# xarray-contrib/xeofs

Hardware: AMD Instinct MI355X
Metric: EOF randomized-SVD GB/s (algorithmic: 16 passes x n x p x 4 B per fit / fit time) (higher is better)
Workload: dtype f32 data, split-fp16 MFMA (f16x3+f16x3), f32 accumulate

## Files before the change

xeofs_amd/csrc/eofx_abi.hip:

```cpp
#include <chrono>
#include "eofx_hfft.hpp"
#include "eofx_kernels.hpp"
#include "eofx_fit.hpp"
#include "eofx_gram.hpp"
#include "eofx_axb_dma.hpp"
#include "eofx_hosteig.hpp"
#include "eofx_hostla.hpp"
#include "eofx_lag.hpp"
#include "eofx_gw.hpp"
#include "eofx_spca.hpp"
#include "eofx_lagcov.hpp"
#include "eofx_lowpass.hpp"
#include "eofx_orderpos.hpp"
#include "eofx_colquad.hpp"
#include "eofx_pairmin.hpp"
#include "eofx_simplex.hpp"
#include "eofx_spectral.hpp"
#include "eofx_pcmul.hpp"
#include "eofx_viewcov.hpp"
#include "eofx_lrfill.hpp"
#include "eofx_plans.hpp"
#include "eofx_sketch.hpp"
#include "eofx_hilbert_host.hpp"
#include "eofx_gwplan.hpp"
// ... 806 lines not shown
#undef EOFX_AXB_ARGS
    KCHK();
  }
  if (ctx->profile) {
    HIPCHK(hipEventRecord(ev1, ctx->stream));
    ctx->prof_events.emplace_back(ev0, ev1, 1);
    ctx->prof_flops += 2.0 * (double)K * (double)rows_pad * (double)L;
    ctx->prof_bytes += (double)K * (double)rows * 4.0 * tiles.columns();
  }
  if (plan.S > 1) {
    const int64_t count4 = rows_pad * L / 4;
    hipLaunchKernelGGL(splitk_reduce_kernel, dim3((int)std::min<int64_t>((count4 + 255) / 256, amax_out ? 2048 : 4096)), dim3(256), 0,
                       ctx->stream, out, W, count4, plan.S, amax_out);
    KCHK();
  }
  return EOFX_OK;
}

static int launch_gram(eofx_ctx* ctx, const float* P, int64_t rows, int L, double* G) {
  const int nb = (L + 63) / 64;
  const int nbx = gram_parts(rows, L);
  ArenaScope scope(ctx);
  ARENA(double, part, (size_t)nbx * L * L);
  hipLaunchKernelGGL(gram_mfma_kernel, dim3(nbx, nb * nb), dim3(256), 0, ctx->stream, P, rows, L, part);
  KCHK();
  const int64_t count = (int64_t)L * L;
  hipLaunchKernelGGL(f64_reduce_kernel, dim3((int)((count + 63) / 64)), dim3(256), 0, ctx->stream,
                     part, G, count, nbx);
  KCHK();
  return EOFX_OK;
}
static int launch_matmul(eofx_ctx* ctx, const float* P, int64_t rows, int L, const double* Mx, int Lo,
                         float* out, bool upper = false, int64_t planes_rows = 0, float planes_bound = 0.f) {
  int KW = (int)std::min<int64_t>(round_up(L, 64), 256);
  if (L > 256) {
    static const int kw_env = std::getenv("EOFX_PMM_KW") ? atoi(std::getenv("EOFX_PMM_KW")) : 0;
    if (kw_env == 128 || kw_env == 256) KW = kw_env;
  }
  const size_t smem = (size_t)KW * PMM_LD * sizeof(double);
  if (smem > 64 * 1024)
    HIPCHK(hipFuncSetAttribute(reinterpret_cast<const void*>(panel_matmul_kernel<false>), hipFuncAttributeMaxDynamicSharedMemorySize, (int)smem));
  const int64_t units = (rows + 127) / 128;
  const int64_t gx = L <= KW ? std::min<int64_t>(units, 1024) : units;
  dim3 grid((int)std::max<int64_t>(1, gx), (Lo + 63) / 64);
  unsigned* amax_out = amax_new(ctx, out);
  if (planes_rows > 0 && Lo == L && amax_out && planes_rows % AXB_KG == 0 && planes_rows <= rows && rows % 8 == 0 && planes_bound > 0.f &&
      std::isfinite(planes_bound) && axb_planes_reserve(ctx, axb_planes_bytes(planes_rows, Lo))) {
    if (smem > 64 * 1024)
      HIPCHK(hipFuncSetAttribute(reinterpret_cast<const void*>(panel_matmul_kernel<false, true>), hipFuncAttributeMaxDynamicSharedMemorySize,
                                 (int)smem));
    hipLaunchKernelGGL((panel_matmul_kernel<false, true>), grid, dim3(256), smem, ctx->stream, P, rows, L, Mx, Lo, out, KW, amax_out,
                       (int64_t)0, (int64_t)0, 1, (const float*)nullptr, upper ? 1 : 0, ctx->axb_planes, planes_rows, planes_bound);
    KCHK();
    ctx->planes_known.panel = out;
    ctx->planes_known.L = Lo;
    ctx->planes_known.K_all = planes_rows;
    ctx->planes_known.bound = planes_bound;
    ctx->planes_known.f32 = true;
    ++ctx->plane_produced[1];
    return EOFX_OK;
  }
  hipLaunchKernelGGL(panel_matmul_kernel<false>, grid, dim3(256), smem, ctx->stream, P, rows, L, Mx, Lo, out, KW, amax_out,
                     (int64_t)0, (int64_t)0, 1, (const float*)nullptr, upper ? 1 : 0);
  KCHK();
  return EOFX_OK;
}
static int launch_matmul_gen(eofx_ctx* ctx, const float* P, int64_t ldp, int64_t slab, int cpb, int64_t rows, int L, const double* Mx, int Lo,
                             const float* sub, float* out) {
  const int KW = (int)std::min<int64_t>(round_up(L, 64), 256);
  const size_t smem = (size_t)KW * PMM_LD * sizeof(double);
  if (smem > 64 * 1024)
    HIPCHK(hipFuncSetAttribute(reinterpret_cast<const void*>(panel_matmul_kernel<true>), hipFuncAttributeMaxDynamicSharedMemorySize, (int)smem));
  const int64_t units = (rows + 127) / 128;
  const int64_t gx = L <= KW ? std::min<int64_t>(units, 1024) : units;
  dim3 grid((int)std::max<int64_t>(1, gx), (Lo + 63) / 64);
  hipLaunchKernelGGL(panel_matmul_kernel<true>, grid, dim3(256), smem, ctx->stream, P, rows, L, Mx, Lo, out, KW, amax_new(ctx, out), ldp,
                     slab, cpb, sub);
  KCHK();
  return EOFX_OK;
}
static int launch_xgram(eofx_ctx* ctx, const float* Pa, int64_t lda, int La, const float* Pb, int64_t ldb, int Lb, int64_t rows, double* C) {
  const int nbx = (int)std::max<int64_t>(1, std::min<int64_t>((rows + 127) / 128, std::max<int64_t>(1, ((int64_t)32 << 20) / ((int64_t)La * Lb * 8))));
  ArenaScope scope(ctx);
  ARENA(double, part, (size_t)nbx * La * Lb);
  hipLaunchKernelGGL(xgram_mfma_kernel, dim3(nbx, (La / 64) * (Lb / 64)), dim3(256), 0, ctx->stream, Pa, lda, Pb, ldb, rows, La, Lb, part);
  KCHK();
// ... 981 lines not shown
    return set_err(ctx, EOFX_ERR_ARG, "import: L=%d must be a positive multiple of 4, l=%d and rows=%lld non-negative", L, l, (long long)rows);
  ENTER(ctx);
  CHK(arena_reserve(ctx, (size_t)rows * l * sizeof(float) + 8192));
  return import_panel(ctx, src, rows, l, P, rows_pad, L);
}

struct LinOp {
  int64_t tall, small, tall_pad, small_pad;
  std::function<int(const float*, float*, int, int)> fwd;
  std::function<int(const float*, float*, int, int)> bwd;
  std::function<int(const float*, float*, int, int, bool)> fwd_to_bwd;
  std::function<int64_t(int, int)> bwd_plane_rows;
  std::function<int(double*, int64_t)> reduce_tall_gram;
  std::function<int(double*, int64_t)> reduce_small_gram;
  int64_t rule_tall_pad = 0;
};

struct RsvdOut {
  float* Tvec;
  float* Svec;
  int Lo;
  std::vector<double> s;
  int64_t tall_pad = 0, small_pad = 0;
};

extern "C" int eofx_orth_tall_rule(int64_t tall_rows_pad, int L, int prec_power) {
  return orth_tall_rule(tall_rows_pad, L, prec_power) ? 1 : 0;
}
extern "C" int eofx_peaked_spectrum(const double* G, int ld, int l) {
  if (!G || l <= 0) return 0;
  std::vector<double> A((size_t)l * l), w(l), V((size_t)l * l);
  for (int i = 0; i < l; ++i)
    for (int j = 0; j < l; ++j) A[(size_t)i * l + j] = 0.5 * (G[(size_t)i * ld + j] + G[(size_t)j * ld + i]);
  for (double v : A)
    if (!std::isfinite(v)) return 0;
  if (eofx_host_eigh_f64(A.data(), l, w.data(), V.data()) != EOFX_OK) return 1;
  if (!(w[0] > 0.0)) return 0;
  return hostla::peaked_spectrum(w.data(), l) ? 1 : 0;
}

static int launch_rinv_blocked(eofx_ctx* ctx, const double* G, int L, int l, double* Rinv) {
  const int Lb = (int)round_up(l, 64), nb = Lb / 64;
  ArenaScope scope(ctx);
  ARENA(double, S, (size_t)Lb * Lb);
  ARENA(double, X, (size_t)Lb * Lb);
  ARENA(double, T, (size_t)Lb * Lb / 2 + 64 * 64);
// ... 74 lines not shown
  }
  return EOFX_OK;
}

constexpr int EOFX_FIT_FALLBACK = 1;
typedef std::function<int(const float*, float*, int)> FirstFwd;
typedef std::function<int(const float*, float*, int)> RangeFinder;
static int rsvd_core(eofx_ctx* ctx, const LinOp& op, int k, int l, int n_iter, const float* omega,
                     RsvdOut& out, const FirstFwd* first_fwd = nullptr, const RangeFinder* range = nullptr) {
  const int L = (int)round_up(l, 32);
  const int Lo = (int)round_up(k, 32);
  AmaxScope amax_scope(ctx);
  ARENA(float, Zs, (size_t)op.small_pad * L);
  ARENA(float, Ws, (size_t)op.small_pad * L);
  ARENA(float, Yt, (size_t)op.tall_pad * L);
  ARENA(float, Qt, (size_t)op.tall_pad * L);
  ARENA(float, Tv, (size_t)op.tall_pad * Lo);
  ARENA(float, Sv, (size_t)op.small_pad * Lo);
  ARENA(double, G, (size_t)L * L);
  ARENA(double, G0, (size_t)L * L);
  ARENA(double, R2, (size_t)L * L);
  ARENA(double, Md, (size_t)L * Lo);
  ARENA(double, Md2, (size_t)L * Lo);
  double* pin = nullptr;
  CHK(pinned_scratch(ctx, &pin));
  if ((size_t)2 * L * L > EOFX_PINNED_DOUBLES) return set_err(ctx, EOFX_ERR_ARG, "internal: sketch too wide for the host scratch");

  CHK(import_panel(ctx, omega, op.small, l, Zs, op.small_pad, L));
  bool first_done = false;
  auto fwd = [&](const float* z, float* y, int prec, int to_bwd = 0) -> int {
    if (first_fwd && !first_done) {
      first_done = true;
      return (*first_fwd)(z, y, L);
    }
    first_done = true;
    if (to_bwd && op.fwd_to_bwd) return op.fwd_to_bwd(z, y, L, prec, to_bwd == 1);
    return op.fwd(z, y, L, prec);
  };
  auto gram_tall = [&](const float* Pn, double* Gout) -> int {
    CHK(launch_gram(ctx, Pn, op.tall_pad, L, Gout));
    return op.reduce_tall_gram ? op.reduce_tall_gram(Gout, (int64_t)L * L) : EOFX_OK;
  };
  auto gram_small = [&](const float* Pn, double* Gout) -> int {
    CHK(launch_gram(ctx, Pn, op.small_pad, L, Gout));
    return op.reduce_small_gram ? op.reduce_small_gram(Gout, (int64_t)L * L) : EOFX_OK;
  };
// ... 61 lines not shown
                       "SVD failed. This may be due to isolated NaN values in the data.");
      Gl[(size_t)i * l + j] = v;
    }
  eofx_host_eigh_f64(Gl.data(), l, w.data(), Uh.data());
  out.s.assign(k, 0.0);
  std::vector<double> M1((size_t)L * Lo, 0.0), M2((size_t)L * Lo, 0.0);
  std::vector<double> invs(k);
  for (int j = 0; j < k; ++j) {
    const double sv = std::sqrt(std::max(w[j], 0.0));
    out.s[j] = sv;
    invs[j] = sv > 0.0 ? 1.0 / sv : 0.0;
  }
  for (int i = 0; i < l; ++i) {
    double* m1 = &M1[(size_t)i * Lo];
    for (int q = 0; q < l; ++q) {
      const double r = hR2[(size_t)i * L + q];
      const double* uq = &Uh[(size_t)q * l];
      for (int j = 0; j < k; ++j) m1[j] += r * uq[j];
    }
    for (int j = 0; j < k; ++j) M2[(size_t)i * Lo + j] = Uh[(size_t)i * l + j] * invs[j];
  }
  HIPCHK(hipMemcpyAsync(Md, M1.data(), sizeof(double) * L * Lo, hipMemcpyHostToDevice, ctx->stream));
  HIPCHK(hipMemcpyAsync(Md2, M2.data(), sizeof(double) * L * Lo, hipMemcpyHostToDevice, ctx->stream));
  CHK(launch_matmul(ctx, Qt, op.tall_pad, L, Md, Lo, Tv));
  CHK(launch_matmul(ctx, Ws, op.small_pad, L, Md2, Lo, Sv));
  HIPCHK(hipStreamSynchronize(ctx->stream));
  out.Tvec = Tv;
  out.Svec = Sv;
  out.Lo = Lo;
  out.tall_pad = op.tall_pad;
  out.small_pad = op.small_pad;
  return EOFX_OK;
}

static int comm_allreduce(eofx_ctx* ctx, void* buf, int64_t count, int dtype, int op);
static int sign_rule(eofx_ctx* ctx, const float* Vpanel, int64_t rows, int Lo, int k,
                     std::vector<double>& sign, bool over_ranks = false) {
  ArenaScope scope(ctx);
  ARENA(float, mx, 2 * (size_t)Lo);
  float* mn = mx + Lo;
  CHK(launch_colminmax(ctx, Vpanel, rows, Lo, mx, mn));
  if (over_ranks) {
    hipLaunchKernelGGL(negate_kernel, dim3(1), dim3(256), 0, ctx->stream, mn, Lo);
    KCHK();
    CHK(comm_allreduce(ctx, mx, 2 * (int64_t)Lo, 0, 1));
  }
  std::vector<float> hmx(Lo), hmn(Lo);
  HIPCHK(hipMemcpyAsync(hmx.data(), mx, sizeof(float) * Lo, hipMemcpyDeviceToHost, ctx->stream));
  HIPCHK(hipMemcpyAsync(hmn.data(), mn, sizeof(float) * Lo, hipMemcpyDeviceToHost, ctx->stream));
  HIPCHK(hipStreamSynchronize(ctx->stream));
  sign.assign(k, 1.0);
  for (int j = 0; j < k; ++j) sign[j] = (std::fabs(hmx[j]) >= std::fabs(hmn[j])) ? 1.0 : -1.0;
  return EOFX_OK;
}

typedef std::function<int(double*, int64_t)> GramReduce;
static int fix_null_columns(eofx_ctx* ctx, float* P, int64_t rows, int64_t rows_pad, int Lo, int k, int first,
                            const GramReduce* reduce = nullptr, int64_t rows_total = -1) {
  if (rows_total < 0) rows_total = rows;
  if (first >= k || rows_total <= first) return EOFX_OK;
  if (!reduce) {
    if (ctx->arena_size - ctx->arena_off < null_repair_bytes(rows_pad, Lo)) return EOFX_OK;
  }
  ArenaScope scope(ctx);
  ARENA(double, G, (size_t)Lo * Lo);
  ARENA(double, Mx, (size_t)Lo * Lo);
  ARENA(float, tmp, (size_t)rows_pad * Lo);
  ARENA(int, dflag, Lo);
  std::vector<double> hG((size_t)Lo * Lo), hM((size_t)Lo * Lo);
  std::vector<int> flag(Lo, 0);
  const int blocks = (int)std::max<int64_t>(1, std::min<int64_t>((rows + 255) / 256, 4096));
  auto gram = [&]() -> int {
    CHK(launch_gram(ctx, P, rows_pad, Lo, G));
// ... 10 lines not shown
    return EOFX_OK;
  };
  int rounds_done = 0;
  for (int attempt = 0; attempt < 8 && rounds_done < 2; ++attempt) {
    CHK(gram());
    const int verdict = hostla::null_column_transform(hG.data(), Lo, first, k, rounds_done == 0, hM.data(), flag.data());
    if (verdict != hostla::NULLCOL_OK) {
      if (rounds_done > 0) break;
      CHK(refill());
      continue;
    }
    HIPCHK(hipMemcpyAsync(Mx, hM.data(), sizeof(double) * Lo * Lo, hipMemcpyHostToDevice, ctx->stream));
    CHK(launch_matmul(ctx, P, rows_pad, Lo, Mx, Lo, tmp));
    HIPCHK(hipMemcpy2DAsync(P + first, sizeof(float) * Lo, tmp + first, sizeof(float) * Lo, sizeof(float) * (size_t)(k - first), (size_t)rows_pad,
                            hipMemcpyDeviceToDevice, ctx->stream));
    HIPCHK(hipStreamSynchronize(ctx->stream));
    ++rounds_done;
  }
  return EOFX_OK;
}

static int fix_null_modes(eofx_ctx* ctx, const RsvdOut& ro, int64_t tall, int64_t small, int k,
                          const GramReduce* reduce_tall = nullptr, int64_t tall_total = -1,
                          const GramReduce* reduce_small = nullptr, int64_t small_total = -1) {
  int first_null = k;
  const double s0 = ro.s.empty() ? 0.0 : ro.s[0];
  for (int j = k - 1; j >= 0 && !(ro.s[j] > 1e-5 * s0); --j) first_null = j;
  if (first_null < k && s0 >= 0.0 && std::isfinite(s0) && ro.tall_pad >= tall && ro.small_pad >= small) {
    CHK(fix_null_columns(ctx, ro.Tvec, tall, ro.tall_pad, ro.Lo, k, first_null, reduce_tall, tall_total));
    CHK(fix_null_columns(ctx, ro.Svec, small, ro.small_pad, ro.Lo, k, first_null, reduce_small, small_total));
  }
  return EOFX_OK;
}

struct FactorShards {
  const GramReduce* reduce_tall = nullptr;
  int64_t tall_total = -1;
  const GramReduce* reduce_small = nullptr;
  int64_t small_total = -1;
};
static int rsvd_finish(eofx_ctx* ctx, const RsvdOut& ro, bool right_is_tall, int64_t left_rows, int64_t right_rows, int k, int flip,
                       float* left, float* s, float* right, double s_divisor = 1.0, const FactorShards* shards = nullptr,
                       std::vector<double>* sign_out = nullptr) {
  const int64_t tall = right_is_tall ? right_rows : left_rows, small = right_is_tall ? left_rows : right_rows;
  const FactorShards local, &sh = shards ? *shards : local;
  CHK(fix_null_modes(ctx, ro, tall, small, k, sh.reduce_tall, sh.tall_total, sh.reduce_small, sh.small_total));
  const float* Rp = right_is_tall ? ro.Tvec : ro.Svec;
  const float* Lp = right_is_tall ? ro.Svec : ro.Tvec;
  std::vector<double> sign;
  if (flip) CHK(sign_rule(ctx, Rp, right_rows, ro.Lo, k, sign, shards != nullptr));
  CHK(export_panel(ctx, Lp, left_rows, ro.Lo, k, flip ? sign.data() : nullptr, left));
  CHK(export_panel(ctx, Rp, right_rows, ro.Lo, k, flip ? sign.data() : nullptr, right));
  if (s) {
    std::vector<float> hs(k);
    for (int j = 0; j < k; ++j) hs[j] = (float)(ro.s[j] / s_divisor);
    HIPCHK(hipMemcpy(s, hs.data(), sizeof(float) * k, hipMemcpyDefault));
  }
  HIPCHK(hipStreamSynchronize(ctx->stream));
  if (sign_out) sign_out->swap(sign);
  return EOFX_OK;
}

static const float* identity_sketch(int64_t small, int l, std::vector<float>& eye) {
  eye.assign((size_t)small * l, 0.f);
  for (int64_t i = 0; i < l; ++i) eye[(size_t)i * l + i] = 1.f;
  return eye.data();
}

extern "C" int eofx_rsvd_f32(eofx_ctx* ctx, const eofx_mat* m, int k, int n_oversamples, int n_iter,
                             const float* omega, int flip, float* U, float* s, float* V) {
  if (!ctx || !m || !omega || k <= 0 || n_oversamples < 0) return set_err(ctx, EOFX_ERR_ARG, "bad argument");
  ENTER(ctx);
  const int64_t n = m->n, p = m->p;
// ... 3523 lines not shown
```

xeofs_amd/csrc/eofx_kernels.hpp:

```cpp
#pragma once
#include <hip/hip_runtime.h>
#include <stdint.h>

#include "eofx_mfma64.hpp"
#include "eofx_plans.hpp"

namespace eofx {

typedef float f32x16 __attribute__((ext_vector_type(16)));
typedef float f32x4 __attribute__((ext_vector_type(4)));
typedef float f32x2 __attribute__((ext_vector_type(2)));

__device__ __forceinline__ void aff_split(double sh, float& hi, float& lo) {
  hi = (float)sh;
  lo = (float)(sh - (double)hi);
}
__device__ __forceinline__ float aff_map(float x, float sh_hi, float sh_lo, float scale) {
  return ((x - sh_hi) - sh_lo) * scale;
}
__device__ __forceinline__ float aff_fma(float x, float sh_hi, float s, float nls) {
  return __builtin_fmaf(x - sh_hi, s, nls);
}

__device__ __forceinline__ void amax_commit(float mx, unsigned* __restrict__ amax_out) {
// ... 968 lines not shown
    f32x4 o = {(float)s0, (float)s1, (float)s2, (float)s3};
    reinterpret_cast<f32x4*>(out)[i] = o;
    mx = fmaxf(mx, fmaxf(fmaxf(fabsf(o[0]), fabsf(o[1])), fmaxf(fabsf(o[2]), fabsf(o[3]))));
  }
  if (amax_out) amax_commit(mx, amax_out);
}

__global__ __launch_bounds__(256) void symmetrize_lower_kernel(float* __restrict__ C, int64_t n, int64_t ld) {
  __shared__ float T[64][65];
  const int bi = blockIdx.y, bj = blockIdx.x;
  if (bj > bi) return;
  const int tx = threadIdx.x & 63, ty = threadIdx.x >> 6;
  for (int r = ty; r < 64; r += 4) {
    const int64_t gr = (int64_t)bj * 64 + r, gc = (int64_t)bi * 64 + tx;
    T[r][tx] = (gr < n && gc < n) ? C[gr * ld + gc] : 0.f;
  }
  __syncthreads();
  for (int r = ty; r < 64; r += 4) {
    const int64_t gr = (int64_t)bi * 64 + r, gc = (int64_t)bj * 64 + tx;
    if (gr < n && gc < n && gc < gr) C[gr * ld + gc] = T[tx][r];
  }
}

__global__ __launch_bounds__(256) void gram_mfma_kernel(const float* __restrict__ P, int64_t rows, int L,
                                                         double* __restrict__ Gpart) {
  const int nb = (L + 63) / 64;
  const int bi = blockIdx.y / nb, bj = blockIdx.y % nb;
  if (bi > bj) return;
  const int wave = threadIdx.x >> 6;
  const Mfma64Lane ln = mfma64_lane();
  const int ca = 64 * bi + 4 * ln.c, cb = 64 * bj + 4 * ln.c;
  const bool same = (bi == bj);
  f64x4 acc[4][4];
  mfma64_zero(acc);
  const int64_t wstride = (int64_t)gridDim.x * 4 * 4;
  auto fetch = [&](int64_t r0, f32x4& va, f32x4& vb) {
    const int64_t r = r0 + ln.k;
    va = f32x4{0.f, 0.f, 0.f, 0.f};
    vb = va;
    if (r < rows) {
      if (ca < L) va = *reinterpret_cast<const f32x4*>(P + r * L + ca);
      if (!same && cb < L) vb = *reinterpret_cast<const f32x4*>(P + r * L + cb);
    }
    if (same) vb = va;
  };
  constexpr int GRAM_PF = 4;
  int64_t r0 = ((int64_t)blockIdx.x * 4 + wave) * 4;
  f32x4 pa[GRAM_PF], pb[GRAM_PF];
#pragma unroll
  for (int d = 0; d < GRAM_PF; ++d) fetch(r0 + d * wstride, pa[d], pb[d]);
  for (; r0 < rows; r0 += GRAM_PF * wstride) {
#pragma unroll
    for (int d = 0; d < GRAM_PF; ++d) {
      const f32x4 va = pa[d], vb = pb[d];
      fetch(r0 + (GRAM_PF + d) * wstride, pa[d], pb[d]);
      __builtin_amdgcn_sched_barrier(0);
      const double a[4] = {(double)va[0], (double)va[1], (double)va[2], (double)va[3]};
      const double b[4] = {(double)vb[0], (double)vb[1], (double)vb[2], (double)vb[3]};
      if (same)
        mfma64_step(acc, a, b, [](int x, int y) { return y >= x; });
      else
        mfma64_step(acc, a, b, Mfma64All{});
    }
  }
  __shared__ double Gs[64][65];
  for (int w = 0; w < 4; ++w) {
    if (wave == w)
      mfma64_each_interleaved(acc, [&](int x, int y) { return !(same && x > y); },
                              [&](int x, int y, int i, int j, double v) {
                                if (w == 0) {
                                  Gs[i][j] = v;
                                  if (same && x < y) Gs[j][i] = v;
                                } else {
                                  Gs[i][j] += v;
                                  if (same && x < y) Gs[j][i] += v;
                                }
                              });
    __syncthreads();
  }
  double* G = Gpart + (int64_t)blockIdx.x * (int64_t)L * L;
  for (int e = threadIdx.x; e < 64 * 64; e += 256) {
    const int i = e >> 6, j = e & 63;
    const int gi = 64 * bi + i, gj = 64 * bj + j;
    if (gi < L && gj < L) {
      G[(int64_t)gi * L + gj] = Gs[i][j];
// ... 281 lines not shown
}

__global__ void chol_blocked_init_kernel(const double* __restrict__ G, int L, int l, double* __restrict__ S, int Lb,
                                          double* __restrict__ d0) {
  const int64_t total = (int64_t)Lb * Lb;
  for (int64_t i = (int64_t)blockIdx.x * blockDim.x + threadIdx.x; i < total; i += (int64_t)gridDim.x * blockDim.x) {
    const int r = (int)(i / Lb), c = (int)(i % Lb);
    double v = (r == c) ? 1.0 : 0.0;
    if (r < l && c < l) v = G[(int64_t)r * L + c];
    S[i] = v;
    if (r == c) d0[r] = v;
  }
}
__global__ void chol_blocked_export_kernel(const double* __restrict__ X, int Lb, int l, double* __restrict__ Rinv, int L) {
  const int64_t total = (int64_t)L * L;
  for (int64_t i = (int64_t)blockIdx.x * blockDim.x + threadIdx.x; i < total; i += (int64_t)gridDim.x * blockDim.x) {
    const int r = (int)(i / L), c = (int)(i % L);
    Rinv[i] = (r <= c && c < l) ? X[(int64_t)r * Lb + c] : 0.0;
  }
}

constexpr int PMM_LD = 66;

template <bool GEN = false, bool PLANES = false>
__global__ __launch_bounds__(256) void panel_matmul_kernel(const float* __restrict__ P,
                                                           int64_t rows, int L,
                                                           const double* __restrict__ Mx, int Lo,
                                                           float* __restrict__ out, int KW,
                                                           unsigned* __restrict__ amax_out = nullptr,
                                                           int64_t ldp = 0, int64_t slab = 0, int cpb = 1,
                                                           const float* __restrict__ sub = nullptr, int upper = 0,
                                                           void* __restrict__ planes = nullptr, int64_t plane_rows = 0,
                                                           float plane_bound = 0.f) {
  static_assert(!(GEN && PLANES), "the plane epilogue belongs to the plain form");
  extern __shared__ __attribute__((aligned(16))) double Ms[];
  float amx = 0.f;
  const int tid = threadIdx.x;
  const int lane = tid & 63, wave = tid >> 6;
  const int li = lane & 15, lk = lane >> 4;
  const int by = upper ? (int)(gridDim.y - 1 - blockIdx.y) : (int)blockIdx.y;
  const int c0 = by * 64;
  const int Lc_all = (L + 63) / 64;
  const int Lc = upper ? (Lc_all < by + 1 ? Lc_all : by + 1) : Lc_all;
  const int Le = L < 64 * Lc ? L : 64 * Lc;
  const int64_t ngroups = (rows + 31) / 32;
  const int64_t g0 = (int64_t)blockIdx.x * 4 + wave;
  auto stage = [&](int k0) {
    for (int i = tid; i < KW * 64; i += 256) {
      const int r = i >> 6, c = i & 63;
      Ms[r * PMM_LD + c] = (k0 + r < L && c0 + c < Lo) ? Mx[(int64_t)(k0 + r) * Lo + c0 + c] : 0.0;
    }
  };
  auto fetch = [&](bool valid, int64_t g, int kc, f32x4 (&a)[2][4]) {
#pragma unroll
    for (int t = 0; t < 2; ++t) {
      const int64_t r = 32 * g + (PLANES ? 8 * (li & 3) + 4 * t + (li >> 2) : 16 * t + li);
#pragma unroll
      for (int tt = 0; tt < 4; ++tt) {
        const int k = kc + 16 * tt + 4 * lk;
        if constexpr (GEN)
          a[t][tt] = (valid && r < rows && k < L) ? *reinterpret_cast<const f32x4*>(P + (int64_t)((k >> 6) / cpb) * slab + ((k >> 6) % cpb) * 64 + r * ldp + (k & 63))
                                                 : f32x4{0.f, 0.f, 0.f, 0.f};
        else
          a[t][tt] = (valid && r < rows && k < L) ? *reinterpret_cast<const f32x4*>(P + r * L + k)
                                                 : f32x4{0.f, 0.f, 0.f, 0.f};
      }
    }
  };
  f64x4 acc[2][4];
  auto compute = [&](int64_t g, int kc, int ms0, const f32x4 (&a)[2][4]) {
    if (kc == 0) {
#pragma unroll
      for (int t = 0; t < 2; ++t)
#pragma unroll
        for (int q = 0; q < 4; ++q) acc[t][q] = f64x4{0.0, 0.0, 0.0, 0.0};
    }
#pragma unroll
    for (int tt = 0; tt < 4; ++tt)
#pragma unroll
      for (int c = 0; c < 4; ++c) {
        double b[4];
#pragma unroll
        for (int q = 0; q < 4; ++q) b[q] = Ms[(kc - ms0 + 16 * tt + 4 * lk + c) * PMM_LD + 16 * q + li];
#pragma unroll
        for (int t = 0; t < 2; ++t)
#pragma unroll
          for (int q = 0; q < 4; ++q)
            acc[t][q] = __builtin_amdgcn_mfma_f64_16x16x4f64((double)a[t][tt][c], b[q], acc[t][q], 0, 0, 0);
      }
    if (kc + 64 >= Le) {
#pragma unroll
      for (int t = 0; t < 2; ++t)
#pragma unroll
        for (int r = 0; r < 4; ++r) {
          const int64_t row = 32 * g + (PLANES ? 8 * lk + 4 * t + r : 16 * t + lk + 4 * r);
          if (row >= rows) continue;
#pragma unroll
          for (int q = 0; q < 4; ++q) {
            const int col = c0 + 16 * q + li;
            if (col < Lo) {
              float o_ = (float)acc[t][q][r];
              if constexpr (GEN) {
                if (sub) o_ = (float)((double)sub[row * Lo + col] - acc[t][q][r]);
              }
              out[row * Lo + col] = o_;
              amx = fmaxf(amx, fabsf(o_));
            }
          }
        }
      if constexpr (PLANES) {
        const int64_t k = 32 * g + 8 * lk;
        if (k < plane_rows) {
          const float p_scale = f16_scale_for(plane_bound);
          float m1 = -1.f;
          asm volatile("" : "+v"(m1));
#pragma unroll
          for (int q = 0; q < 4; ++q) {
            const int col = c0 + 16 * q + li;
            u32x4 hi, lo;
#pragma unroll
            for (int t = 0; t < 2; ++t)
#pragma unroll
              for (int r = 0; r < 4; r += 2) {
                const bool in_ = col < Lo && k + 4 * t + r < rows;
                const float v0 = (in_ ? (float)acc[t][q][r] : 0.f) * p_scale;
                const float v1 = (in_ ? (float)acc[t][q][r + 1] : 0.f) * p_scale;
                const fp16x2_t h = cvt_pk_rn(v0, v1);
                fp16x2_t l;
                l[0] = (__fp16)__builtin_fmaf((float)h[0], m1, v0);
// ... 23 lines not shown
      if (item + 1 < nitems) {
        fetch(item + 2 < nitems, g0 + ((item + 2) / Lc) * gstride, (int)((item + 2) % Lc) * 64, a0);
        __builtin_amdgcn_sched_barrier(0);
        compute(g0 + ((item + 1) / Lc) * gstride, (int)((item + 1) % Lc) * 64, 0, a1);
      }
    }
  } else {
    const bool active = g0 < ngroups;
    const int wc = KW / 64;
    fetch(active, g0, 0, a0);
    for (int w0 = 0; w0 < Lc; w0 += wc) {
      __syncthreads();
      stage(64 * w0);
      __syncthreads();
      const int we = w0 + wc < Lc ? w0 + wc : Lc;
      for (int ch = w0; ch < we; ch += 2) {
        fetch(active && ch + 1 < Lc, g0, 64 * (ch + 1), a1);
        __builtin_amdgcn_sched_barrier(0);
        if (active) compute(g0, 64 * ch, 64 * w0, a0);
        fetch(active && ch + 2 < Lc, g0, 64 * (ch + 2), a0);
        __builtin_amdgcn_sched_barrier(0);
        if (active && ch + 1 < we) compute(g0, 64 * (ch + 1), 64 * w0, a1);
      }
    }
  }
  if constexpr (PLANES) {
    if (amax_out && blockIdx.x == 0 && blockIdx.y == 0 && tid == 0) *amax_out = __float_as_uint(plane_bound);
  } else if (amax_out) {
    amax_commit(amx, amax_out);
  }
}

__global__ __launch_bounds__(256) void colminmax_part_kernel(const float* __restrict__ P,
                                                             int64_t rows, int L,
                                                             float* __restrict__ pmx,
                                                             float* __restrict__ pmn) {
  __shared__ float smx[16][64], smn[16][64];
  const int tid = threadIdx.x;
  const int cq = tid & 15, rl = tid >> 4;
  const int c = blockIdx.y * 64 + 4 * cq;
  f32x4 mx = {-INFINITY, -INFINITY, -INFINITY, -INFINITY}, mn = {INFINITY, INFINITY, INFINITY, INFINITY};
  if (c < L) {
    const int64_t step = (int64_t)gridDim.x * 16;
    int64_t r = (int64_t)blockIdx.x * 16 + rl;
    for (; r + 7 * step < rows; r += 8 * step) {
      f32x4 v[8];
// ... 1131 lines not shown
```

xeofs_amd/csrc/eofx_plans.hpp:

```cpp
#pragma once
#include <algorithm>
#include <cmath>
#include <cstddef>
#include <cstdint>
#include <cstdlib>
#include <vector>

#include "eofx.h"

namespace eofx {

constexpr int ATB_KG = 32;
constexpr int ATB_BM = 512;
constexpr int AXB_KG = 64;
constexpr int AXB_BM = 256;
constexpr int GR_BM = 256;
constexpr int GR_BK = 32;
constexpr int64_t EOFX_GRAM_MAX_SIDE = 32768;
constexpr int SPCA_GMAX = 2048;
constexpr int VIEWCOV_T = 128;
constexpr int VIEWCOV_K = 16;
constexpr int VIEWCOV_WGS = 512;
constexpr int VIEWCOV_SPLIT_SLABS = 16;
constexpr int FIR_R = 64;
// ... 3 lines not shown
constexpr int LAGCOV_PMAX = 1024;
constexpr int LAGCOV_FUSE_NTAU = 65;
constexpr int LAGCOV_WGS = 512;
constexpr int LOWPASS_WGS = 512;
constexpr int64_t LOWPASS_PART_MAX = (int64_t)1 << 23;
constexpr int EOFX_LAG_GROUP_COLS = 1024;

inline int64_t round_up(int64_t x, int64_t m) { return (x + m - 1) / m * m; }

#if defined(__HIPCC__)
#define EOFX_HOST_DEVICE __host__ __device__
#else
#define EOFX_HOST_DEVICE
#endif
constexpr int AXB_PLANE_BYTES = 8 * 64 * 16;
constexpr int AXB_PAIR_BYTES = 2 * AXB_PLANE_BYTES;
EOFX_HOST_DEVICE inline int64_t axb_plane_offset(int64_t cb, int64_t K_all, int64_t k, int c, int plane) {
  const int64_t pair = k >> 6;
  const int g = (int)(k >> 3) & 7, t = (int)k & 7;
  const int slot = c ^ ((c >> 3) & 7);
  return (cb * (K_all / AXB_KG) + pair) * AXB_PAIR_BYTES + (int64_t)plane * AXB_PLANE_BYTES + (g * 64 + slot) * 16 + t * 2;
}
inline size_t axb_planes_bytes(int64_t K_all, int L) { return (size_t)((L + 63) / 64) * (size_t)(K_all / AXB_KG) * AXB_PAIR_BYTES; }

struct AtbPlan {
  int S;
  int64_t kps;
};
inline bool atb_wide(int L) {
  if (const char* ev = std::getenv("EOFX_ATB_WIDE_MIN")) return L >= atoi(ev);
  return L >= 96;
}
inline AtbPlan atb_plan(int64_t M, int64_t K, int L, bool wide = false) {
  const int bx = (int)(M / ATB_BM);
  const int bz = wide ? (L + 127) / 128 : (L + 63) / 64;
  const double resident = wide ? 256.0 : 512.0;
  AtbPlan best{1, K};
  if (const char* ev = std::getenv("EOFX_ATB_SPLITS"))
    if (atoi(ev) == 1) return best;
  double best_t = 1e30;
  for (int S = 1; S <= 128; ++S) {
    const int64_t kps = round_up((K + S - 1) / S, ATB_KG);
    const int s_eff = (int)((K + kps - 1) / kps);
    if (s_eff != S) continue;
    const double blocks = (double)bx * bz * s_eff;
    const double rounds = std::ceil(blocks / resident);
// ... 431 lines not shown
```

Measured before the change: 5987.

## Fuse column extrema into panel matmul, add triangular k-skip and single-block gram path

Three separate changes. The final panel matmul can now track per-column min/max during its epilogue and reduce them with atomics into 16 key sets, so the sign rule no longer needs a separate colminmax pass over the tall panel. A triangular mode skips MFMA work on the zero half of upper-triangular multipliers, and the single-block (L<=64) gram kernel gets a self-product variant with a deeper prefetch. The costs are extra atomics and registers in the epilogue and more template instantiations.

After: 6011 (median of 6 runs). Within noise of the previous version (+0.4%).

```diff
diff --git a/xeofs_amd/csrc/eofx_abi.hip b/xeofs_amd/csrc/eofx_abi.hip
--- a/xeofs_amd/csrc/eofx_abi.hip
+++ b/xeofs_amd/csrc/eofx_abi.hip
@@ -852,7 +852,9 @@
   const int nbx = gram_parts(rows, L);
   ArenaScope scope(ctx);
   ARENA(double, part, (size_t)nbx * L * L);
-  hipLaunchKernelGGL(gram_mfma_kernel, dim3(nbx, nb * nb), dim3(256), 0, ctx->stream, P, rows, L, part);
+  const int depth = nb == 1 ? gram64_depth() : 4;
+  const auto kern = depth == 16 ? gram_mfma_kernel<16> : depth == 8 ? gram_mfma_kernel<8> : gram_mfma_kernel<0>;
+  hipLaunchKernelGGL(kern, dim3(nbx, nb * nb), dim3(256), 0, ctx->stream, P, rows, L, part);
   KCHK();
   const int64_t count = (int64_t)L * L;
   hipLaunchKernelGGL(f64_reduce_kernel, dim3((int)((count + 63) / 64)), dim3(256), 0, ctx->stream,
@@ -861,26 +863,31 @@
   return EOFX_OK;
 }
 static int launch_matmul(eofx_ctx* ctx, const float* P, int64_t rows, int L, const double* Mx, int Lo,
-                         float* out, bool upper = false, int64_t planes_rows = 0, float planes_bound = 0.f) {
+                         float* out, bool upper = false, int64_t planes_rows = 0, float planes_bound = 0.f, unsigned* ext = nullptr,
+                         int64_t ext_rows = 0) {
+  if (ext && (upper || planes_rows > 0)) return set_err(ctx, EOFX_ERR_ARG, "internal: column extrema belong to the plain product");
   int KW = (int)std::min<int64_t>(round_up(L, 64), 256);
   if (L > 256) {
     static const int kw_env = std::getenv("EOFX_PMM_KW") ? atoi(std::getenv("EOFX_PMM_KW")) : 0;
     if (kw_env == 128 || kw_env == 256) KW = kw_env;
   }
   const size_t smem = (size_t)KW * PMM_LD * sizeof(double);
-  if (smem > 64 * 1024)
-    HIPCHK(hipFuncSetAttribute(reinterpret_cast<const void*>(panel_matmul_kernel<false>), hipFuncAttributeMaxDynamicSharedMemorySize, (int)smem));
   const int64_t units = (rows + 127) / 128;
   const int64_t gx = L <= KW ? std::min<int64_t>(units, 1024) : units;
   dim3 grid((int)std::max<int64_t>(1, gx), (Lo + 63) / 64);
   unsigned* amax_out = amax_new(ctx, out);
-  if (planes_rows > 0 && Lo == L && amax_out && planes_rows % AXB_KG == 0 && planes_rows <= rows && rows % 8 == 0 && planes_bound > 0.f &&
-      std::isfinite(planes_bound) && axb_planes_reserve(ctx, axb_planes_bytes(planes_rows, Lo))) {
-    if (smem > 64 * 1024)
-      HIPCHK(hipFuncSetAttribute(reinterpret_cast<const void*>(panel_matmul_kernel<false, true>), hipFuncAttributeMaxDynamicSharedMemorySize,
-                                 (int)smem));
-    hipLaunchKernelGGL((panel_matmul_kernel<false, true>), grid, dim3(256), smem, ctx->stream, P, rows, L, Mx, Lo, out, KW, amax_out,
-                       (int64_t)0, (int64_t)0, 1, (const float*)nullptr, upper ? 1 : 0, ctx->axb_planes, planes_rows, planes_bound);
+  const bool planes = planes_rows > 0 && Lo == L && amax_out && planes_rows % AXB_KG == 0 && planes_rows <= rows && rows % 8 == 0 &&
+                      planes_bound > 0.f && std::isfinite(planes_bound) && axb_planes_reserve(ctx, axb_planes_bytes(planes_rows, Lo));
+  const bool tri = upper && pmm_tri_mode() == 2;
+  const auto kern = planes ? (tri ? panel_matmul_kernel<false, true, true> : panel_matmul_kernel<false, true>)
+                    : tri  ? panel_matmul_kernel<false, false, true>
+                    : ext  ? panel_matmul_kernel<false, false, false, true>
+                           : panel_matmul_kernel<false>;
+  if (smem > 64 * 1024)
+    HIPCHK(hipFuncSetAttribute(reinterpret_cast<const void*>(kern), hipFuncAttributeMaxDynamicSharedMemorySize, (int)smem));
+  if (planes) {
+    hipLaunchKernelGGL(kern, grid, dim3(256), smem, ctx->stream, P, rows, L, Mx, Lo, out, KW, amax_out, (int64_t)0, (int64_t)0, 1,
+                       (const float*)nullptr, upper ? 1 : 0, (void*)ctx->axb_planes, planes_rows, planes_bound, (unsigned*)nullptr, (int64_t)0);
     KCHK();
     ctx->planes_known.panel = out;
     ctx->planes_known.L = Lo;
@@ -890,8 +897,8 @@
     ++ctx->plane_produced[1];
     return EOFX_OK;
   }
-  hipLaunchKernelGGL(panel_matmul_kernel<false>, grid, dim3(256), smem, ctx->stream, P, rows, L, Mx, Lo, out, KW, amax_out,
-                     (int64_t)0, (int64_t)0, 1, (const float*)nullptr, upper ? 1 : 0);
+  hipLaunchKernelGGL(kern, grid, dim3(256), smem, ctx->stream, P, rows, L, Mx, Lo, out, KW, amax_out, (int64_t)0, (int64_t)0, 1,
+                     (const float*)nullptr, upper ? 1 : 0, (void*)nullptr, (int64_t)0, 0.f, ext, ext_rows);
   KCHK();
   return EOFX_OK;
 }
@@ -1919,6 +1926,8 @@
   int Lo;
   std::vector<double> s;
   int64_t tall_pad = 0, small_pad = 0;
+  const unsigned* tall_ext = nullptr;
+  int64_t tall_ext_rows = 0;
 };
 
 extern "C" int eofx_orth_tall_rule(int64_t tall_rows_pad, int L, int prec_power) {
@@ -2039,6 +2048,7 @@
   ARENA(double, R2, (size_t)L * L);
   ARENA(double, Md, (size_t)L * Lo);
   ARENA(double, Md2, (size_t)L * Lo);
+  ARENA(unsigned, Tv_ext, (size_t)PMM_EXT_SETS * 2 * Lo);
   double* pin = nullptr;
   CHK(pinned_scratch(ctx, &pin));
   if ((size_t)2 * L * L > EOFX_PINNED_DOUBLES) return set_err(ctx, EOFX_ERR_ARG, "internal: sketch too wide for the host scratch");
@@ -2146,7 +2156,11 @@
   }
   HIPCHK(hipMemcpyAsync(Md, M1.data(), sizeof(double) * L * Lo, hipMemcpyHostToDevice, ctx->stream));
   HIPCHK(hipMemcpyAsync(Md2, M2.data(), sizeof(double) * L * Lo, hipMemcpyHostToDevice, ctx->stream));
-  CHK(launch_matmul(ctx, Qt, op.tall_pad, L, Md, Lo, Tv));
+  const bool with_ext = pmm_extrema_on();
+  std::vector<unsigned> ext_init((size_t)PMM_EXT_SETS * 2 * Lo);
+  for (size_t i = 0; i < ext_init.size(); ++i) ext_init[i] = (i / Lo) % 2 == 0 ? F32_KEY_NEG_INF : F32_KEY_POS_INF;
+  if (with_ext) HIPCHK(hipMemcpyAsync(Tv_ext, ext_init.data(), sizeof(unsigned) * ext_init.size(), hipMemcpyHostToDevice, ctx->stream));
+  CHK(launch_matmul(ctx, Qt, op.tall_pad, L, Md, Lo, Tv, false, 0, 0.f, with_ext ? Tv_ext : nullptr, op.tall));
   CHK(launch_matmul(ctx, Ws, op.small_pad, L, Md2, Lo, Sv));
   HIPCHK(hipStreamSynchronize(ctx->stream));
   out.Tvec = Tv;
@@ -2154,25 +2168,54 @@
   out.Lo = Lo;
   out.tall_pad = op.tall_pad;
   out.small_pad = op.small_pad;
+  out.tall_ext = with_ext ? Tv_ext : nullptr;
+  out.tall_ext_rows = op.tall;
   return EOFX_OK;
 }
 
 static int comm_allreduce(eofx_ctx* ctx, void* buf, int64_t count, int dtype, int op);
 static int sign_rule(eofx_ctx* ctx, const float* Vpanel, int64_t rows, int Lo, int k,
-                     std::vector<double>& sign, bool over_ranks = false) {
-  ArenaScope scope(ctx);
-  ARENA(float, mx, 2 * (size_t)Lo);
-  float* mn = mx + Lo;
-  CHK(launch_colminmax(ctx, Vpanel, rows, Lo, mx, mn));
-  if (over_ranks) {
-    hipLaunchKernelGGL(negate_kernel, dim3(1), dim3(256), 0, ctx->stream, mn, Lo);
-    KCHK();
-    CHK(comm_allreduce(ctx, mx, 2 * (int64_t)Lo, 0, 1));
-  }
+                     std::vector<double>& sign, bool over_ranks = false, const unsigned* ext = nullptr) {
+  ArenaScope scope(ctx);
   std::vector<float> hmx(Lo), hmn(Lo);
-  HIPCHK(hipMemcpyAsync(hmx.data(), mx, sizeof(float) * Lo, hipMemcpyDeviceToHost, ctx->stream));
-  HIPCHK(hipMemcpyAsync(hmn.data(), mn, sizeof(float) * Lo, hipMemcpyDeviceToHost, ctx->stream));
-  HIPCHK(hipStreamSynchronize(ctx->stream));
+  if (ext && !over_ranks) {
+    std::vector<unsigned> key((size_t)PMM_EXT_SETS * 2 * Lo);
+    HIPCHK(hipMemcpyAsync(key.data(), ext, sizeof(unsigned) * key.size(), hipMemcpyDeviceToHost, ctx->stream));
+    HIPCHK(hipStreamSynchronize(ctx->stream));
+    for (int j = 0; j < Lo; ++j) {
+      unsigned ka = key[j], kb = key[(size_t)Lo + j];
+      for (int t = 1; t < PMM_EXT_SETS; ++t) {
+        ka = std::max(ka, key[(size_t)t * 2 * Lo + j]);
+        kb = std::min(kb, key[(size_t)t * 2 * Lo + Lo + j]);
+      }
+      const unsigned a = f32_order_unkey(ka), b = f32_order_unkey(kb);
+      std::memcpy(&hmx[j], &a, sizeof(float));
+      std::memcpy(&hmn[j], &b, sizeof(float));
+    }
+    if (pmm_extrema_mode() == 2) {
+      ARENA(float, mx, 2 * (size_t)Lo);
+      std::vector<float> chk(2 * (size_t)Lo);
+      CHK(launch_colminmax(ctx, Vpanel, rows, Lo, mx, mx + Lo));
+      HIPCHK(hipMemcpyAsync(chk.data(), mx, sizeof(float) * 2 * Lo, hipMemcpyDeviceToHost, ctx->stream));
+      HIPCHK(hipStreamSynchronize(ctx->stream));
+      for (int j = 0; j < Lo; ++j)
+        if (!(chk[j] == hmx[j]) || !(chk[(size_t)Lo + j] == hmn[j]))
+          return set_err(ctx, EOFX_ERR_ARG, "internal: column extrema of the product differ from those of the panel: column %d, max %.9g / %.9g, min %.9g / %.9g", j,
+                         (double)hmx[j], (double)chk[j], (double)hmn[j], (double)chk[(size_t)Lo + j]);
+    }
+  } else {
+    ARENA(float, mx, 2 * (size_t)Lo);
+    float* mn = mx + Lo;
+    CHK(launch_colminmax(ctx, Vpanel, rows, Lo, mx, mn));
+    if (over_ranks) {
+      hipLaunchKernelGGL(negate_kernel, dim3(1), dim3(256), 0, ctx->stream, mn, Lo);
+      KCHK();
+      CHK(comm_allreduce(ctx, mx, 2 * (int64_t)Lo, 0, 1));
+    }
+    HIPCHK(hipMemcpyAsync(hmx.data(), mx, sizeof(float) * Lo, hipMemcpyDeviceToHost, ctx->stream));
+    HIPCHK(hipMemcpyAsync(hmn.data(), mn, sizeof(float) * Lo, hipMemcpyDeviceToHost, ctx->stream));
+    HIPCHK(hipStreamSynchronize(ctx->stream));
+  }
   sign.assign(k, 1.0);
   for (int j = 0; j < k; ++j) sign[j] = (std::fabs(hmx[j]) >= std::fabs(hmn[j])) ? 1.0 : -1.0;
   return EOFX_OK;
@@ -2229,11 +2272,12 @@
 
 static int fix_null_modes(eofx_ctx* ctx, const RsvdOut& ro, int64_t tall, int64_t small, int k,
                           const GramReduce* reduce_tall = nullptr, int64_t tall_total = -1,
-                          const GramReduce* reduce_small = nullptr, int64_t small_total = -1) {
+                          const GramReduce* reduce_small = nullptr, int64_t small_total = -1, bool* repaired = nullptr) {
   int first_null = k;
   const double s0 = ro.s.empty() ? 0.0 : ro.s[0];
   for (int j = k - 1; j >= 0 && !(ro.s[j] > 1e-5 * s0); --j) first_null = j;
   if (first_null < k && s0 >= 0.0 && std::isfinite(s0) && ro.tall_pad >= tall && ro.small_pad >= small) {
+    if (repaired) *repaired = true;
     CHK(fix_null_columns(ctx, ro.Tvec, tall, ro.tall_pad, ro.Lo, k, first_null, reduce_tall, tall_total));
     CHK(fix_null_columns(ctx, ro.Svec, small, ro.small_pad, ro.Lo, k, first_null, reduce_small, small_total));
   }
@@ -2251,11 +2295,13 @@
                        std::vector<double>* sign_out = nullptr) {
   const int64_t tall = right_is_tall ? right_rows : left_rows, small = right_is_tall ? left_rows : right_rows;
   const FactorShards local, &sh = shards ? *shards : local;
-  CHK(fix_null_modes(ctx, ro, tall, small, k, sh.reduce_tall, sh.tall_total, sh.reduce_small, sh.small_total));
+  bool repaired = false;
+  CHK(fix_null_modes(ctx, ro, tall, small, k, sh.reduce_tall, sh.tall_total, sh.reduce_small, sh.small_total, &repaired));
   const float* Rp = right_is_tall ? ro.Tvec : ro.Svec;
   const float* Lp = right_is_tall ? ro.Svec : ro.Tvec;
   std::vector<double> sign;
-  if (flip) CHK(sign_rule(ctx, Rp, right_rows, ro.Lo, k, sign, shards != nullptr));
+  const unsigned* ext = right_is_tall && !repaired && !shards && ro.tall_ext_rows == right_rows ? ro.tall_ext : nullptr;
+  if (flip) CHK(sign_rule(ctx, Rp, right_rows, ro.Lo, k, sign, shards != nullptr, ext));
   CHK(export_panel(ctx, Lp, left_rows, ro.Lo, k, flip ? sign.data() : nullptr, left));
   CHK(export_panel(ctx, Rp, right_rows, ro.Lo, k, flip ? sign.data() : nullptr, right));
   if (s) {
diff --git a/xeofs_amd/csrc/eofx_kernels.hpp b/xeofs_amd/csrc/eofx_kernels.hpp
--- a/xeofs_amd/csrc/eofx_kernels.hpp
+++ b/xeofs_amd/csrc/eofx_kernels.hpp
@@ -1014,15 +1014,16 @@
   }
 }
 
+template <int ONE = 0>
 __global__ __launch_bounds__(256) void gram_mfma_kernel(const float* __restrict__ P, int64_t rows, int L,
                                                          double* __restrict__ Gpart) {
-  const int nb = (L + 63) / 64;
+  const int nb = ONE ? 1 : (L + 63) / 64;
   const int bi = blockIdx.y / nb, bj = blockIdx.y % nb;
   if (bi > bj) return;
   const int wave = threadIdx.x >> 6;
   const Mfma64Lane ln = mfma64_lane();
   const int ca = 64 * bi + 4 * ln.c, cb = 64 * bj + 4 * ln.c;
-  const bool same = (bi == bj);
+  const bool same = ONE ? true : (bi == bj);
   f64x4 acc[4][4];
   mfma64_zero(acc);
   const int64_t wstride = (int64_t)gridDim.x * 4 * 4;
@@ -1036,23 +1037,43 @@
     }
     if (same) vb = va;
   };
-  constexpr int GRAM_PF = 4;
+  constexpr int GRAM_PF = ONE ? ONE : 4;
   int64_t r0 = ((int64_t)blockIdx.x * 4 + wave) * 4;
-  f32x4 pa[GRAM_PF], pb[GRAM_PF];
-#pragma unroll
-  for (int d = 0; d < GRAM_PF; ++d) fetch(r0 + d * wstride, pa[d], pb[d]);
-  for (; r0 < rows; r0 += GRAM_PF * wstride) {
-#pragma unroll
-    for (int d = 0; d < GRAM_PF; ++d) {
-      const f32x4 va = pa[d], vb = pb[d];
-      fetch(r0 + (GRAM_PF + d) * wstride, pa[d], pb[d]);
-      __builtin_amdgcn_sched_barrier(0);
-      const double a[4] = {(double)va[0], (double)va[1], (double)va[2], (double)va[3]};
-      const double b[4] = {(double)vb[0], (double)vb[1], (double)vb[2], (double)vb[3]};
-      if (same)
-        mfma64_step(acc, a, b, [](int x, int y) { return y >= x; });
-      else
-        mfma64_step(acc, a, b, Mfma64All{});
+  if constexpr (ONE > 0) {
+    f32x4 pa[GRAM_PF];
+    auto fetch1 = [&](int64_t rr, f32x4& va) {
+      const int64_t r = rr + ln.k;
+      va = (r < rows && ca < L) ? *reinterpret_cast<const f32x4*>(P + r * L + ca) : f32x4{0.f, 0.f, 0.f, 0.f};
+    };
+#pragma unroll
+    for (int d = 0; d < GRAM_PF; ++d) fetch1(r0 + d * wstride, pa[d]);
+    for (; r0 < rows; r0 += GRAM_PF * wstride) {
+#pragma unroll
+      for (int d = 0; d < GRAM_PF; ++d) {
+        const f32x4 va = pa[d];
+        fetch1(r0 + (GRAM_PF + d) * wstride, pa[d]);
+        __builtin_amdgcn_sched_barrier(0);
+        const double a[4] = {(double)va[0], (double)va[1], (double)va[2], (double)va[3]};
+        mfma64_step(acc, a, a, [](int x, int y) { return y >= x; });
+      }
+    }
+  } else {
+    f32x4 pa[GRAM_PF], pb[GRAM_PF];
+#pragma unroll
+    for (int d = 0; d < GRAM_PF; ++d) fetch(r0 + d * wstride, pa[d], pb[d]);
+    for (; r0 < rows; r0 += GRAM_PF * wstride) {
+#pragma unroll
+      for (int d = 0; d < GRAM_PF; ++d) {
+        const f32x4 va = pa[d], vb = pb[d];
+        fetch(r0 + (GRAM_PF + d) * wstride, pa[d], pb[d]);
+        __builtin_amdgcn_sched_barrier(0);
+        const double a[4] = {(double)va[0], (double)va[1], (double)va[2], (double)va[3]};
+        const double b[4] = {(double)vb[0], (double)vb[1], (double)vb[2], (double)vb[3]};
+        if (same)
+          mfma64_step(acc, a, b, [](int x, int y) { return y >= x; });
+        else
+          mfma64_step(acc, a, b, Mfma64All{});
+      }
     }
   }
   __shared__ double Gs[64][65];
@@ -1380,7 +1401,7 @@
 
 constexpr int PMM_LD = 66;
 
-template <bool GEN = false, bool PLANES = false>
+template <bool GEN = false, bool PLANES = false, bool TRI = false, bool EXT = false>
 __global__ __launch_bounds__(256) void panel_matmul_kernel(const float* __restrict__ P,
                                                            int64_t rows, int L,
                                                            const double* __restrict__ Mx, int Lo,
@@ -1389,8 +1410,11 @@
                                                            int64_t ldp = 0, int64_t slab = 0, int cpb = 1,
                                                            const float* __restrict__ sub = nullptr, int upper = 0,
                                                            void* __restrict__ planes = nullptr, int64_t plane_rows = 0,
-                                                           float plane_bound = 0.f) {
+                                                           float plane_bound = 0.f, unsigned* __restrict__ ext = nullptr,
+                                                           int64_t ext_rows = 0) {
   static_assert(!(GEN && PLANES), "the plane epilogue belongs to the plain form");
+  static_assert(!(EXT && (GEN || PLANES)), "the extrema epilogue belongs to the plain form without planes");
+  static_assert(!(GEN && TRI), "the k-step rule belongs to the plain form");
   extern __shared__ __attribute__((aligned(16))) double Ms[];
   float amx = 0.f;
   const int tid = threadIdx.x;
@@ -1426,6 +1450,7 @@
     }
   };
   f64x4 acc[2][4];
+  float emx[4] = {-INFINITY, -INFINITY, -INFINITY, -INFINITY}, emn[4] = {INFINITY, INFINITY, INFINITY, INFINITY};
   auto compute = [&](int64_t g, int kc, int ms0, const f32x4 (&a)[2][4]) {
     if (kc == 0) {
 #pragma unroll
@@ -1433,19 +1458,44 @@
 #pragma unroll
         for (int q = 0; q < 4; ++q) acc[t][q] = f64x4{0.0, 0.0, 0.0, 0.0};
     }
-#pragma unroll
-    for (int tt = 0; tt < 4; ++tt)
-#pragma unroll
-      for (int c = 0; c < 4; ++c) {
-        double b[4];
-#pragma unroll
-        for (int q = 0; q < 4; ++q) b[q] = Ms[(kc - ms0 + 16 * tt + 4 * lk + c) * PMM_LD + 16 * q + li];
-#pragma unroll
-        for (int t = 0; t < 2; ++t)
-#pragma unroll
-          for (int q = 0; q < 4; ++q)
-            acc[t][q] = __builtin_amdgcn_mfma_f64_16x16x4f64((double)a[t][tt][c], b[q], acc[t][q], 0, 0, 0);
-      }
+    if constexpr (TRI) {
+      const int chunk = kc >> 6;
+      const bool diag = pmm_tri_last_kstep(by, 0, chunk) < 3;
+#pragma unroll
+      for (int tt = 0; tt < 4; ++tt) {
+#pragma unroll
+        for (int part = 0; part < 2; ++part) {
+          const int q0 = part == 0 ? tt : 0, q1 = part == 0 ? 4 : tt;
+          if (part == 1 && (tt == 0 || diag)) continue;
+#pragma unroll
+          for (int c = 0; c < 4; ++c) {
+            double b[4];
+#pragma unroll
+            for (int q = 0; q < 4; ++q)
+              if (q >= q0 && q < q1) b[q] = Ms[(kc - ms0 + 16 * tt + 4 * lk + c) * PMM_LD + 16 * q + li];
+#pragma unroll
+            for (int t = 0; t < 2; ++t)
+#pragma unroll
+              for (int q = 0; q < 4; ++q)
+                if (q >= q0 && q < q1) acc[t][q] = __builtin_amdgcn_mfma_f64_16x16x4f64((double)a[t][tt][c], b[q], acc[t][q], 0, 0, 0);
+          }
+        }
+      }
+    } else {
+#pragma unroll
+      for (int tt = 0; tt < 4; ++tt)
+#pragma unroll
+        for (int c = 0; c < 4; ++c) {
+          double b[4];
+#pragma unroll
+          for (int q = 0; q < 4; ++q) b[q] = Ms[(kc - ms0 + 16 * tt + 4 * lk + c) * PMM_LD + 16 * q + li];
+#pragma unroll
+          for (int t = 0; t < 2; ++t)
+#pragma unroll
+            for (int q = 0; q < 4; ++q)
+              acc[t][q] = __builtin_amdgcn_mfma_f64_16x16x4f64((double)a[t][tt][c], b[q], acc[t][q], 0, 0, 0);
+        }
+    }
     if (kc + 64 >= Le) {
 #pragma unroll
       for (int t = 0; t < 2; ++t)
@@ -1463,6 +1513,12 @@
               }
               out[row * Lo + col] = o_;
               amx = fmaxf(amx, fabsf(o_));
+              if constexpr (EXT) {
+                if (row < ext_rows && o_ == o_) {
+                  emx[q] = fmaxf(emx[q], o_);
+                  emn[q] = fminf(emn[q], o_);
+                }
+              }
             }
           }
         }
@@ -1532,6 +1588,35 @@
         __builtin_amdgcn_sched_barrier(0);
         if (active && ch + 1 < we) compute(g0, 64 * (ch + 1), 64 * w0, a1);
       }
+    }
+  }
+  if constexpr (EXT) {
+#pragma unroll
+    for (int q = 0; q < 4; ++q) {
+      emx[q] = fmaxf(emx[q], __shfl_xor(emx[q], 16));
+      emx[q] = fmaxf(emx[q], __shfl_xor(emx[q], 32));
+      emn[q] = fminf(emn[q], __shfl_xor(emn[q], 16));
+      emn[q] = fminf(emn[q], __shfl_xor(emn[q], 32));
+    }
+    __syncthreads();
+    float* Es = reinterpret_cast<float*>(Ms);
+    if (lk == 0) {
+#pragma unroll
+      for (int q = 0; q < 4; ++q) {
+        Es[wave * 128 + 16 * q + li] = emx[q];
+        Es[wave * 128 + 64 + 16 * q + li] = emn[q];
+      }
+    }
+    __syncthreads();
+    if (tid < 128 && c0 + (tid & 63) < Lo) {
+      const bool is_min = tid >= 64;
+      float v = Es[tid];
+#pragma unroll
+      for (int w = 1; w < 4; ++w) v = is_min ? fminf(v, Es[w * 128 + tid]) : fmaxf(v, Es[w * 128 + tid]);
+      const unsigned key = f32_order_key(__float_as_uint(v));
+      unsigned* set = ext + (size_t)(blockIdx.x % PMM_EXT_SETS) * 2 * Lo;
+      if (is_min) atomicMin(set + Lo + c0 + (tid & 63), key);
+      else atomicMax(set + c0 + (tid & 63), key);
     }
   }
   if constexpr (PLANES) {
diff --git a/xeofs_amd/csrc/eofx_plans.hpp b/xeofs_amd/csrc/eofx_plans.hpp
--- a/xeofs_amd/csrc/eofx_plans.hpp
+++ b/xeofs_amd/csrc/eofx_plans.hpp
@@ -49,6 +49,29 @@
   return (cb * (K_all / AXB_KG) + pair) * AXB_PAIR_BYTES + (int64_t)plane * AXB_PLANE_BYTES + (g * 64 + slot) * 16 + t * 2;
 }
 inline size_t axb_planes_bytes(int64_t K_all, int L) { return (size_t)((L + 63) / 64) * (size_t)(K_all / AXB_KG) * AXB_PAIR_BYTES; }
+
+EOFX_HOST_DEVICE inline int pmm_tri_last_kstep(int by, int q, int chunk) { return chunk < by ? 3 : chunk == by ? q : -1; }
+inline int pmm_tri_mode() {
+  const char* ev = std::getenv("EOFX_PMM_TRI_KSTEPS");
+  return ev && atoi(ev) == 0 ? 1 : 2;
+}
+EOFX_HOST_DEVICE inline unsigned f32_order_key(unsigned bits) { return (bits & 0x80000000u) ? ~bits : bits | 0x80000000u; }
+EOFX_HOST_DEVICE inline unsigned f32_order_unkey(unsigned key) { return (key & 0x80000000u) ? key ^ 0x80000000u : ~key; }
+constexpr int PMM_EXT_SETS = 16;
+constexpr unsigned F32_KEY_NEG_INF = 0x007FFFFFu, F32_KEY_POS_INF = 0xFF800000u;
+inline int pmm_extrema_mode() {
+  const char* ev = std::getenv("EOFX_PMM_EXTREMA");
+  return !ev ? 1 : atoi(ev) == 0 ? 0 : atoi(ev) == 2 ? 2 : 1;
+}
+inline bool pmm_extrema_on() { return pmm_extrema_mode() != 0; }
+constexpr int GRAM64_DEPTH = 16;
+inline int gram64_depth() {
+  if (const char* ev = std::getenv("EOFX_GRAM_DEPTH")) {
+    const int d = atoi(ev);
+    if (d == 4 || d == 8 || d == 16) return d;
+  }
+  return GRAM64_DEPTH;
+}
 
 struct AtbPlan {
   int S;
```
